# speechbrain/speechbrain

Measured on AMD Instinct MI355X. Metric: audio-sec/s decoded (node), Conformer-L beam=10, higher is better.
Workload: dtype f32

## Files before the change

speechbrain_amd/csrc/gemm.hip:

```cpp
#include "common.h"
#include "internal.h"

#include <map>
#include <mutex>
#include <type_traits>

namespace {

using sbk::f32x16;

#include "gemm_common.h"

__device__ __forceinline__ void tile_epilogue_32x32(const GemmArgs& g, float (&v)[16], int mt, int nt, int r, int half) {
  const int col = nt * 32 + r;
  const bool col_ok = col < g.N;
  const float bv = (g.bias && col_ok) ? g.bias[col] : 0.0f;
  float res[16];
  int len[16];
#pragma unroll
  for (int q = 0; q < 16; ++q) {
    const int row = mt * 32 + (q & 3) + 8 * (q >> 2) + 4 * half;
    const bool live = col_ok && row < g.M;
    res[q] = (live && g.R) ? g.R[(size_t)row * g.ldr + col] : 0.0f;
    len[q] = (live && g.seq_len) ? g.seq_len[row / g.rows_per_seq] : 0x7fffffff;
// ... 936 lines not shown
    } else {
      SBK_LAUNCH((gemm_skinny_flat_kernel<1>), grid, block, 0, st, g, ws, tiles_m, tiles_n);
    }
  } else if (nch >= 4) {
    SBK_LAUNCH((gemm_skinny_kernel<4>), grid, block, 0, st, g, ws, kper, tiles_m, tiles_n);
  } else if (nch >= 2) {
    SBK_LAUNCH((gemm_skinny_kernel<2>), grid, block, 0, st, g, ws, kper, tiles_m, tiles_n);
  } else {
    SBK_LAUNCH((gemm_skinny_kernel<1>), grid, block, 0, st, g, ws, kper, tiles_m, tiles_n);
  }
  int rc = launch_status("gemm_skinny");
  if (rc || SKg == 1) return rc;
  const size_t total = (size_t)M * N;
  SBK_LAUNCH(splitk_reduce_kernel, dim3((unsigned)((total + 1023) / 1024)), dim3(256), 0, st, g, (const float*)ws, SKg);
  return launch_status("splitk_reduce");
}

int gemm_ln_nt(const float* A, int lda, const float* Wf, int ldw, const float* bf, const float* R, int ldr, float* C,
               int ldc, int M, int N, int K, float eps, int act, float alpha, hipStream_t st) {
  if (M == 0 || N == 0) return 0;
  const bool ok = (K == 512 || K == 256 || K == 128) && (M <= 512 || (long)cdiv(M, 128) * cdiv(N, 128) < 256) &&
                  M <= 4096 && (long)M * N < 1900000 && lda % 4 == 0 && ldw % 4 == 0 && aligned16(A) && aligned16(Wf) &&
                  !g_skinny_off;
  if (!ok) return -1;
  GemmArgs g{A, Wf, bf, R, C, lda, ldw, ldr, ldc, M, N, K, act, alpha, nullptr, 1};
  const int tiles_m = cdiv(M, 32), tiles_n = cdiv(N, 32);
  ProfScope prof("gemm_skinny_ln", 2.0 * M * N * K, 4.0 * ((double)M * K + (double)N * K + (double)M * N), st);
  dim3 grid(8 * tiles_m * cdiv(tiles_n, 8)), block(256);
  if (K == 512) {
    SBK_LAUNCH((gemm_skinny_ln_kernel<4>), grid, block, 0, st, g, eps, tiles_m, tiles_n);
  } else if (K == 256) {
    SBK_LAUNCH((gemm_skinny_ln_kernel<2>), grid, block, 0, st, g, eps, tiles_m, tiles_n);
  } else {
    SBK_LAUNCH((gemm_skinny_ln_kernel<1>), grid, block, 0, st, g, eps, tiles_m, tiles_n);
  }
  return launch_status("gemm_skinny_ln");
}

int g_sk_mode = 1;
int g_sk_min_rows = 2048;
namespace {
constexpr int kSkMaxGrid = 512, kSkMaxTiles = 1 << 16;
int sk_cus();
}
int sk_route(int M, int N, int K, int* bt) {
  int unused;
  if (!bt) bt = &unused;
  *bt = 128;
  if (!g_sk_mode || K % 32 != 0 || K < 64) return 0;
  const long T = (long)cdiv(M, 128) * cdiv(N, 128), U = T * (K / 32);
  const int cus = sk_cus();
  int G = 0;
  if (g_sk_mode == 1 && M < g_sk_min_rows) return 0;
  if (g_sk_mode == 1) {
    const bool narrow_short = N <= 512 && K <= 512;
    if (narrow_short ? 2 * T < 3L * cus : U < 16L * cus) return 0;
    G = U >= 32L * cus ? 2 * cus : cus;
  } else {
    if (g_sk_mode == 3 && T < 8) return 0;
    G = 2 * cus;
    if (U / 4 < G) G = (int)(U / 4);
  }
  if (G > kSkMaxGrid) G = kSkMaxGrid;
  return G >= 8 ? (G / 8) * 8 : 8;
}
namespace {
struct SkWorkspace {
  float* slabs;
  int* cnt;
};
std::mutex g_sk_mu;
std::map<std::pair<int, hipStream_t>, SkWorkspace> g_sk_ws;
int g_sk_cus[64] = {};

int cur_device() {
  int dev = 0;
  (void)hipGetDevice(&dev);
  return dev;
}

constexpr size_t kSkSlabBytes = (size_t)2 * 256 * 256 * 256 * sizeof(float);
static_assert(kSkSlabBytes >= (size_t)2 * kSkMaxGrid * 128 * 128 * sizeof(float), "slab area");
constexpr size_t kSkTicketBytes = (size_t)kSkMaxTiles * sizeof(int);

bool sk_workspace(hipStream_t st, SkWorkspace* out) {
  std::lock_guard<std::mutex> lk(g_sk_mu);
  auto it = g_sk_ws.find(std::make_pair(cur_device(), st));
  if (it == g_sk_ws.end()) return false;
  *out = it->second;
  return true;
}

}
int* tile_tickets(hipStream_t st, long tiles) {
  SkWorkspace w;
  if (tiles > kSkMaxTiles || !sk_workspace(st, &w)) return nullptr;
  return w.cnt;
}
bool stream_ws(hipStream_t st, float** slabs, int** cnt) {
  SkWorkspace w;
  if (!sk_workspace(st, &w)) return false;
  *slabs = w.slabs;
  *cnt = w.cnt;
  return true;
}
namespace {

int sk_cus() {
  const int dev = cur_device() & 63;
  if (!g_sk_cus[dev]) {
    int cus = 0;
    (void)hipDeviceGetAttribute(&cus, hipDeviceAttributeMultiprocessorCount, dev);
    g_sk_cus[dev] = cus > 0 ? cus : 256;
  }
  return g_sk_cus[dev];
}

}
int device_cus() { return sk_cus(); }
namespace {
int launch_sk(const GemmArgs& g, int G, int bt, hipStream_t st, bool x3 = false) {
  SkArgs s;
  s.g = g;
  s.tiles_n = cdiv(g.N, bt);
  s.tiles = cdiv(g.M, bt) * s.tiles_n;
  s.KT = g.K / 32;
  if (s.tiles > kSkMaxTiles || (long)s.tiles * s.KT > (1L << 30)) return -1;
  SkWorkspace w;
  if (!sk_workspace(st, &w)) return -1;
  s.slabs = w.slabs;
  s.cnt = w.cnt;
  const size_t lds = x3 ? (size_t)2 * (128 * 32 + 128 * 48) * sizeof(float) : (size_t)(2 * 2 * bt * 32 + 4) * sizeof(float);
  static bool once = false;
  if (!once) {
    (void)SBK_ALLOW_DYN_LDS((gemm_nt_sk_kernel<128, false>), (size_t)(2 * 2 * 128 * 32 + 4) * sizeof(float));
    (void)SBK_ALLOW_DYN_LDS((gemm_nt_sk_kernel<128, true>), (size_t)2 * (128 * 32 + 128 * 48) * sizeof(float));
    once = true;
  }
  const double flops = 2.0 * g.M * g.N * g.K, bytes = 4.0 * ((double)g.M * g.K + (double)g.N * g.K + (double)g.M * g.N);
  if (x3) {
    ProfScope prof("gemm_nt_f32x3", flops, bytes + 2.0 * (double)g.N * g.K, st);
    SBK_LAUNCH((gemm_nt_sk_kernel<128, true>), dim3((unsigned)G), dim3(256), lds, st, s);
  } else {
    ProfScope prof("gemm_nt_persistent", flops, bytes, st);
    SBK_LAUNCH((gemm_nt_sk_kernel<128, false>), dim3((unsigned)G), dim3(256), lds, st, s);
  }
  return launch_status("sbk_gemm_nt_f32 (stream-K)");
}
}

int g_x3_route_rows = 1024, g_x3_route_tiles = 192;
bool x3_routed(int M, int N, int K) {
  return M >= g_x3_route_rows && K % 32 == 0 && K >= 64 && N % 4 == 0 && (long)cdiv(M, 128) * cdiv(N, 128) >= g_x3_route_tiles;
}

int gemm_nt_x3(const float* A, int lda, const uint16_t* W3, const float* bias, const float* R, int ldr, float* C, int ldc,
               int M, int N, int K, int act, float alpha, const int32_t* seq_len, int rows_per_seq, hipStream_t st) {
  if (M == 0 || N == 0) return 0;
  GemmArgs g{A, reinterpret_cast<const float*>(W3), bias, R, C, lda, 0, ldr, ldc, M, N, K, act, alpha, seq_len,
             rows_per_seq > 0 ? rows_per_seq : 1};
  const long T = (long)cdiv(M, 128) * cdiv(N, 128), U = T * (K / 32);
  const int cus = sk_cus();
  int G = T >= 2L * cus ? 2 * cus : cus;
  if (U / 4 < G) G = (int)(U / 4);
  if (G > kSkMaxGrid) G = kSkMaxGrid;
  G = G >= 8 ? (G / 8) * 8 : 8;
  return launch_sk(g, G, 128, st, true);
}

int gemm_nt(const float* A, int lda, const float* W, int ldw, const float* bias, const float* R, int ldr, float* C,
            int ldc, int M, int N, int K, int act, float alpha, const int32_t* seq_len, int rows_per_seq, hipStream_t st) {
  if (M == 0 || N == 0) return 0;
  GemmArgs g{A, W, bias, R, C, lda, ldw, ldr, ldc, M, N, K, act, alpha, seq_len, rows_per_seq > 0 ? rows_per_seq : 1};
  const bool vec = (lda % 4 == 0) && (ldw % 4 == 0) && aligned16(A) && aligned16(W);
  const long tiles128 = (long)cdiv(M, 128) * cdiv(N, 128);
  const long tiles64 = (long)cdiv(M, 64) * cdiv(N, 64);
  if (vec) {
    int bt = 128;
    const int G = sk_route(M, N, K, &bt);
    if (G > 0) {
      const int rc = launch_sk(g, G, bt, st);
      if (rc != -1) return rc;
    }
  }
  if (tiles128 >= 384) return launch_gemm<128, 128, 32, 64, 64>(g, vec, st);
  if (tiles64 >= 256 || M > 256) return launch_gemm<64, 64, 32, 32, 32>(g, vec, st);
  return launch_gemm<32, 64, 32, 32, 32>(g, vec, st);
}
}

extern "C" size_t sbk_stream_workspace_bytes(void) { return sbk::kSkSlabBytes + sbk::kSkTicketBytes; }

extern "C" int sbk_stream_workspace_set(sbk_stream_t stream, void* workspace, size_t workspace_bytes) {
  SBK_REQUIRE(workspace && ((uintptr_t)workspace & 255) == 0, "stream workspace: null or not 256-byte aligned");
  SBK_REQUIRE(workspace_bytes >= sbk_stream_workspace_bytes(), "stream workspace: %zu bytes given, %zu needed", workspace_bytes,
              sbk_stream_workspace_bytes());
  hipStream_t st = sbk::as_stream(stream);
  sbk::SkWorkspace w{reinterpret_cast<float*>(workspace),
                     reinterpret_cast<int*>(reinterpret_cast<char*>(workspace) + sbk::kSkSlabBytes)};
  const hipError_t e = hipMemsetAsync(w.cnt, 0, sbk::kSkTicketBytes, st);
  if (e != hipSuccess) return sbk::fail((int)e, "stream workspace: memset: %s", hipGetErrorString(e));
  std::lock_guard<std::mutex> lk(sbk::g_sk_mu);
  sbk::g_sk_ws[std::make_pair(sbk::cur_device(), st)] = w;
  return 0;
}

extern "C" int sbk_stream_workspace_release(sbk_stream_t stream) {
  std::lock_guard<std::mutex> lk(sbk::g_sk_mu);
  sbk::g_sk_ws.erase(std::make_pair(sbk::cur_device(), sbk::as_stream(stream)));
  return 0;
}

extern "C" int sbk_gemm_nt_f32(const float* A, int lda, const float* W, int ldw, const float* bias,
                               const float* residual, int ldr, float* C, int ldc, int M, int N, int K, int act,
                               float alpha, const int32_t* seq_len, int rows_per_seq, sbk_stream_t stream) {
  if (M == 0 || N == 0) return 0;
  SBK_REQUIRE(A && W && C, "gemm: null operand");
  SBK_REQUIRE(M >= 0 && N >= 0 && K > 0, "gemm: bad shape M=%d N=%d K=%d", M, N, K);
  SBK_REQUIRE(lda > 0 && ldw >= K && ldc >= N, "gemm: leading dimension smaller than the row");
  SBK_REQUIRE(!residual || ldr >= N, "gemm: residual stride");
  SBK_REQUIRE(act >= SBK_ACT_NONE && act <= SBK_ACT_LEAKY_RELU, "gemm: unknown activation %d", act);
  SBK_REQUIRE(!seq_len || rows_per_seq > 0, "gemm: seq_len given without rows_per_seq");
  return sbk::gemm_nt_ws(A, lda, W, ldw, bias, residual, ldr, C, ldc, M, N, K, act, alpha, seq_len, rows_per_seq,
                         nullptr, 0, sbk::as_stream(stream));
}

extern "C" int sbk_gemm_ln_nt_f32(const float* A, int lda, const float* Wf, int ldw, const float* bf,
                                  const float* residual, int ldr, float* C, int ldc, int M, int N, int K, float eps,
                                  int act, float alpha, sbk_stream_t stream) {
  if (M == 0 || N == 0) return 0;
  SBK_REQUIRE(A && Wf && C, "gemm_ln: null operand");
  SBK_REQUIRE(M >= 0 && N >= 0 && K > 0 && lda >= K && ldw >= K && ldc >= N, "gemm_ln: bad shape");
  const int rc = sbk::gemm_ln_nt(A, lda, Wf, ldw, bf, residual, ldr, C, ldc, M, N, K, eps, act, alpha,
                                 sbk::as_stream(stream));
  if (rc == -1) return sbk::fail(SBK_EINVAL, "gemm_ln: shape M=%d N=%d K=%d not eligible for the fused kernel", M, N, K);
  return rc;
}

extern "C" int sbk_gemm_nt_splitk_f32(const float* A, int lda, const float* W, int ldw, const float* bias,
                                      const float* residual, int ldr, float* C, int ldc, int M, int N, int K, int act,
                                      float alpha, float* workspace, size_t workspace_floats, sbk_stream_t stream) {
  if (M == 0 || N == 0) return 0;
  SBK_REQUIRE(A && W && C, "gemm: null operand");
  SBK_REQUIRE(M >= 0 && N >= 0 && K > 0, "gemm: bad shape M=%d N=%d K=%d", M, N, K);
  SBK_REQUIRE(lda >= K && ldw >= K && ldc >= N, "gemm: leading dimension smaller than the row");
  SBK_REQUIRE(!residual || ldr >= N, "gemm: residual stride");
  SBK_REQUIRE(act >= SBK_ACT_NONE && act <= SBK_ACT_LEAKY_RELU, "gemm: unknown activation %d", act);
  return sbk::gemm_nt_ws(A, lda, W, ldw, bias, residual, ldr, C, ldc, M, N, K, act, alpha, nullptr, 0, workspace,
                         workspace ? workspace_floats : 0, sbk::as_stream(stream));
}


extern "C" int sbk_prof_gemm_repeat_f32(const float* A, const float* W, float* C, int M, int N, int K, float* workspace,
                                        size_t workspace_floats, int iters, float* us_per_launch,
                                        sbk_stream_t stream) {
  SBK_REQUIRE(A && W && C && us_per_launch && iters > 0, "gemm_repeat: bad arguments");
  hipStream_t st = sbk::as_stream(stream);
  hipEvent_t e0, e1;
  if (hipEventCreate(&e0) != hipSuccess || hipEventCreate(&e1) != hipSuccess) return sbk::fail(1, "event create");
  int rc = 0;
  for (int i = 0; i < 3 && !rc; ++i)
    rc = sbk::gemm_nt_ws(A, K, W, K, nullptr, nullptr, 0, C, N, M, N, K, SBK_ACT_NONE, 1.0f, nullptr, 0, workspace,
                         workspace_floats, st);
  (void)hipEventRecord(e0, st);
  for (int i = 0; i < iters && !rc; ++i)
    rc = sbk::gemm_nt_ws(A, K, W, K, nullptr, nullptr, 0, C, N, M, N, K, SBK_ACT_NONE, 1.0f, nullptr, 0, workspace,
                         workspace_floats, st);
  (void)hipEventRecord(e1, st);
  (void)hipEventSynchronize(e1);
  float ms = 0.0f;
  (void)hipEventElapsedTime(&ms, e0, e1);
  *us_per_launch = ms * 1000.0f / iters;
  return rc;
}

static int* knob_slot(int key) {
  switch (key) {
    case 2: return &sbk::g_skinny_off;
    case 4: return &sbk::g_cross_rows;
    case 8: return &sbk::g_cross_fc256;
    case 14: return &sbk::g_tiled_splitk;
    case 18: return &sbk::g_sk_mode;
    case 24: return &sbk::g_sk_min_rows;
    case 34: return &sbk::g_x3_route_rows;
    case 35: return &sbk::g_x3_route_tiles;
    case 40: return &sbk::g_score_fused;
    case 41: return &sbk::g_x3r_mode;
    case 42: return &sbk::g_x3r_min_rows;
    case 45: return &sbk::g_x3r_ln;
    case 47: return &sbk::g_persist;
    case 48: return &sbk::g_persist_grid;
    case 49: return &sbk::g_persist_stamps;
    case 51: return &sbk::g_x3r_xc;
    case 53: return &sbk::g_nt_mask;
    case 54: return &sbk::g_x3r_probe;
    case 55: return &sbk::g_self_anc;
    case 58: return &sbk::g_x3r_pair;
    case 59: return &sbk::g_persist_tree;
    case 60: return &sbk::g_attn_exp2;
    case 61: return &sbk::g_lp256;
    case 62: return &sbk::g_lp256_mode;
    case 63: return &sbk::g_x3p_fast_epi;
    case 64: return &sbk::g_x3p_mode;
    default: return nullptr;
  }
}
extern "C" void sbk_prof_set_knob(int key, int value) {
  if (int* p = knob_slot(key)) *p = value;
}
extern "C" int sbk_prof_get_knob(int key) {
  const int* p = knob_slot(key);
  return p ? *p : (-2147483647 - 1);
}


extern "C" int sbk_split_bf16x3(const float* W, int ldw, uint16_t* W3, int N, int K, sbk_stream_t stream) {
  if (N == 0) return 0;
  SBK_REQUIRE(W && W3 && N > 0 && K > 0 && K % 32 == 0 && ldw >= K, "split_bf16x3: bad arguments (K must be a multiple of 32)");
  const long n = (long)N * K, blocks = (n + 255) / 256;
  SBK_LAUNCH(split_bf16x3_kernel, dim3((unsigned)(blocks < 8192 ? blocks : 8192)), dim3(256), 0, sbk::as_stream(stream), W, ldw,
             reinterpret_cast<unsigned short*>(W3), n, K);
  return sbk::launch_status("sbk_split_bf16x3");
}

extern "C" int sbk_gemm_nt_f32x3(const float* A, int lda, const uint16_t* W3, const float* bias, const float* residual,
                                 int ldr, float* C, int ldc, int M, int N, int K, int act, float alpha,
                                 const int32_t* seq_len, int rows_per_seq, sbk_stream_t stream) {
  if (M == 0 || N == 0) return 0;
  SBK_REQUIRE(A && W3 && C, "gemm_f32x3: null operand");
  SBK_REQUIRE(M >= 0 && N >= 0 && K >= 64 && K % 32 == 0, "gemm_f32x3: bad shape M=%d N=%d K=%d (K: a multiple of 32, >= 64)", M, N, K);
  SBK_REQUIRE(lda > 0 && lda % 4 == 0 && ldc >= N && sbk::aligned16(A) && sbk::aligned16(W3),
              "gemm_f32x3: operand rows must be 16-byte aligned (lda=%d)", lda);
  SBK_REQUIRE(N % 4 == 0 && ldc % 4 == 0 && sbk::aligned16(C) && (!bias || sbk::aligned16(bias)),
              "gemm_f32x3: N and ldc must be multiples of 4, C / bias 16-byte aligned (rows are stored as 16-byte vectors)");
  SBK_REQUIRE(!residual || (ldr >= N && ldr % 4 == 0 && sbk::aligned16(residual)), "gemm_f32x3: residual stride / alignment");
  SBK_REQUIRE(act >= SBK_ACT_NONE && act <= SBK_ACT_LEAKY_RELU, "gemm_f32x3: unknown activation %d", act);
  SBK_REQUIRE(!seq_len || rows_per_seq > 0, "gemm_f32x3: seq_len given without rows_per_seq");
  const int rc = sbk::gemm_nt_x3(A, lda, W3, bias, residual, ldr, C, ldc, M, N, K, act, alpha, seq_len, rows_per_seq,
                                 sbk::as_stream(stream));
  if (rc == -1) return sbk::fail(SBK_EINVAL, "gemm_f32x3: no workspace registered for this stream (sbk_stream_workspace_set) or too many tiles");
  return rc;
}
```

speechbrain_amd/csrc/gemm_x3r.hip:

```cpp
#include "common.h"
#include "internal.h"

namespace {

using sbk::f32x16;

struct X3rArgs {
  const float* A;
  const uint4* PW;
  const float* bias;
  const float* R;
  float* C;
  int ns;
  int lda, ldr, ldc, M, N, K, act, tiles_m, tiles_n;
  float alpha;
  float ln_eps;
  int xc;
};

template <int NS, int LNQ = 0, bool PAIR = false>
__global__ void __launch_bounds__(256, 2) gemm_x3r_kernel(X3rArgs g) {
  constexpr int DEPTH = 4, PD = 3;
  __shared__ float4 red[4][4][4][64];
  __shared__ float2 stat[LNQ > 0 ? 64 : 1];
  const int lane = threadIdx.x & 63, wave = threadIdx.x >> 6;
  int nt, mt;
  {
    const int id = blockIdx.x, x = id & 7, q = id >> 3;
    const int c = g.xc, r = 8 / c, rm = (g.tiles_m + r - 1) / r;
    mt = x / c + r * (q % rm);
    nt = x % c + c * (q / rm);
    if (mt >= g.tiles_m || nt >= g.tiles_n) return;
  }
  const int r = lane & 31, half = lane >> 5;
  const int ns = NS > 0 ? NS : g.ns, k_begin = wave * ns * 16, KB = g.K >> 4;
  const float* arow[2];
#pragma unroll
  for (int i = 0; i < 2; ++i) arow[i] = g.A + (size_t)min(mt * 64 + i * 32 + r, g.M - 1) * g.lda + k_begin + 8 * half;
  const uint4* wp = g.PW + ((size_t)(nt * KB + (k_begin >> 4)) * 6 + half) * 64 + r;
  float4 av[DEPTH][2][2];
  uint4 wv[DEPTH][2][3];
  auto load = [&](int buf, int st) SBK_INLINE_LAMBDA {
#pragma unroll
    for (int j = 0; j < 2; ++j)
#pragma unroll
      for (int p = 0; p < 3; ++p) wv[buf][j][p] = wp[(size_t)st * 384 + p * 128 + j * 32];
#pragma unroll
    for (int i = 0; i < 2; ++i) {
      av[buf][i][0] = *reinterpret_cast<const float4*>(arow[i] + st * 16);
      av[buf][i][1] = *reinterpret_cast<const float4*>(arow[i] + st * 16 + 4);
    }
  };
  f32x16 acc[2][2];
#pragma unroll
  for (int i = 0; i < 2; ++i)
#pragma unroll
    for (int j = 0; j < 2; ++j)
#pragma unroll
      for (int q = 0; q < 16; ++q) acc[i][j][q] = 0.0f;
  float mean[2] = {0.0f, 0.0f};
  auto compute = [&](int buf) SBK_INLINE_LAMBDA {
    sbk::bf16x8 ap[2][3], bp[2][3];
#pragma unroll
    for (int j = 0; j < 2; ++j)
#pragma unroll
      for (int p = 0; p < 3; ++p) {
        sbk::pin(wv[buf][j][p].x), sbk::pin(wv[buf][j][p].y), sbk::pin(wv[buf][j][p].z), sbk::pin(wv[buf][j][p].w);
        const uint4 u = wv[buf][j][p];
        bp[j][p] = sbk::bf16x8_from_words(u.x, u.y, u.z, u.w);
      }
#pragma unroll
    for (int i = 0; i < 2; ++i) {
#pragma unroll
      for (int e = 0; e < 2; ++e) {
        sbk::pin(av[buf][i][e].x), sbk::pin(av[buf][i][e].y), sbk::pin(av[buf][i][e].z), sbk::pin(av[buf][i][e].w);
      }
      const float4 x0 = av[buf][i][0], x1 = av[buf][i][1];
      float x[8] = {x0.x, x0.y, x0.z, x0.w, x1.x, x1.y, x1.z, x1.w};
      if constexpr (LNQ > 0) {
#pragma unroll
        for (int e = 0; e < 8; ++e) x[e] -= mean[i];
      }
      unsigned h[4], m[4], l[4];
#pragma unroll
      for (int p = 0; p < 4; ++p) {
        h[p] = sbk::bf16_pair(x[2 * p], x[2 * p + 1]);
        const float r0 = x[2 * p] - __uint_as_float(h[p] << 16), r1 = x[2 * p + 1] - __uint_as_float(h[p] & 0xffff0000u);
        m[p] = sbk::bf16_pair(r0, r1);
        l[p] = sbk::bf16_pair(r0 - __uint_as_float(m[p] << 16), r1 - __uint_as_float(m[p] & 0xffff0000u));
      }
      ap[i][0] = sbk::bf16x8_from_words(h[0], h[1], h[2], h[3]);
      ap[i][1] = sbk::bf16x8_from_words(m[0], m[1], m[2], m[3]);
      ap[i][2] = sbk::bf16x8_from_words(l[0], l[1], l[2], l[3]);
    }
    constexpr int PA_[6] = {2, 0, 1, 1, 0, 0}, PB_[6] = {0, 2, 1, 0, 1, 0};
#pragma unroll
    for (int t = 0; t < 6; ++t)
#pragma unroll
      for (int i = 0; i < 2; ++i)
#pragma unroll
        for (int j = 0; j < 2; ++j) acc[i][j] = sbk::mfma_32x32x16_bf16(bp[j][PB_[t]], ap[i][PA_[t]], acc[i][j]);
  };
#pragma unroll
  for (int st = 0; st < (PAIR ? DEPTH : PD); ++st) load(st, st);
  if constexpr (LNQ > 0) {
    const float inv_k = 1.0f / (float)g.K;
    const int grp = lane >> 4, t = lane & 15;
#pragma unroll
    for (int ps = 0; ps < 4; ++ps) {
      const int rl = wave * 16 + ps * 4 + grp;
      const float4* xr = reinterpret_cast<const float4*>(g.A + (size_t)min(mt * 64 + rl, g.M - 1) * g.lda);
      float4 xs[4 * LNQ];
#pragma unroll
      for (int j = 0; j < 4 * LNQ; ++j) xs[j] = xr[t + 16 * j];
      float sm = 0.0f;
#pragma unroll
      for (int j = 0; j < 4 * LNQ; ++j) sm += (xs[j].x + xs[j].y) + (xs[j].z + xs[j].w);
      const float mu = sbk::group_sum<16>(sm) * inv_k;
      float qs = 0.0f;
#pragma unroll
      for (int j = 0; j < 4 * LNQ; ++j) {
        const float a = xs[j].x - mu, b = xs[j].y - mu, c = xs[j].z - mu, d = xs[j].w - mu;
        qs += (a * a + b * b) + (c * c + d * d);
      }
      const float rs = rsqrtf(sbk::group_sum<16>(qs) * inv_k + g.ln_eps);
      if (t == 0) stat[rl] = make_float2(mu, rs);
    }
    __syncthreads();
#pragma unroll
    for (int i = 0; i < 2; ++i) mean[i] = stat[i * 32 + r].x;
  }
  if constexpr (PAIR && NS > 0) {
#pragma unroll
    for (int st = 0; st < NS; st += 2) {
      compute(st % DEPTH);
      compute((st + 1) % DEPTH);
      sbk::sched_fence();
      if (st + DEPTH < NS) {
        load(st % DEPTH, st + DEPTH);
        load((st + 1) % DEPTH, st + DEPTH + 1);
      }
      sbk::sched_fence();
    }
  } else if constexpr (PAIR) {
#pragma unroll 1
    for (int s0 = 0; s0 < ns; s0 += DEPTH) {
#pragma unroll
      for (int j = 0; j < DEPTH; j += 2) {
        compute(j);
        compute(j + 1);
        sbk::sched_fence();
        if (s0 + j + DEPTH < ns) {
          load(j, s0 + j + DEPTH);
          load(j + 1, s0 + j + DEPTH + 1);
        }
        sbk::sched_fence();
      }
    }
  } else if constexpr (NS > 0) {
#pragma unroll
    for (int st = 0; st < NS; ++st) {
      if (st + PD < NS) load((st + PD) % DEPTH, st + PD);
      sbk::sched_fence();
      compute(st % DEPTH);
    }
  } else {
#pragma unroll 1
    for (int s0 = 0; s0 < ns; s0 += DEPTH) {
#pragma unroll
      for (int j = 0; j < DEPTH; ++j) {
        if (s0 + j + PD < ns) load((j + PD) % DEPTH, s0 + j + PD);
        sbk::sched_fence();
        compute(j);
      }
    }
  }
  const int row = (mt * 2 + (wave >> 1)) * 32 + r, col0 = (nt * 2 + (wave & 1)) * 32 + 4 * half;
  const bool row_ok = row < g.M;
  const float* rrow = g.R ? g.R + (size_t)(row_ok ? row : 0) * g.ldr : nullptr;
  float4 bv[4], rv[4];
  bool ok[4];
  auto side_loads = [&]() SBK_INLINE_LAMBDA {
#pragma unroll
    for (int q4 = 0; q4 < 4; ++q4) {
      const int col = col0 + 8 * q4;
      ok[q4] = row_ok && col < g.N;
      bv[q4] = (g.bias && ok[q4]) ? *reinterpret_cast<const float4*>(g.bias + col) : make_float4(0.0f, 0.0f, 0.0f, 0.0f);
      rv[q4] = (rrow && ok[q4]) ? *reinterpret_cast<const float4*>(rrow + col) : make_float4(0.0f, 0.0f, 0.0f, 0.0f);
    }
  };
  side_loads();
#pragma unroll
  for (int i = 0; i < 2; ++i)
#pragma unroll
    for (int j = 0; j < 2; ++j)
#pragma unroll
      for (int q4 = 0; q4 < 4; ++q4)
        red[wave][2 * i + j][q4][lane] = make_float4(acc[i][j][4 * q4], acc[i][j][4 * q4 + 1], acc[i][j][4 * q4 + 2], acc[i][j][4 * q4 + 3]);
  __syncthreads();
  float4 v[4];
#pragma unroll
  for (int q4 = 0; q4 < 4; ++q4) {
    const float4 a0 = red[0][wave][q4][lane], a1 = red[1][wave][q4][lane], a2 = red[2][wave][q4][lane], a3 = red[3][wave][q4][lane];
    v[q4] = make_float4(((a0.x + a1.x) + a2.x) + a3.x, ((a0.y + a1.y) + a2.y) + a3.y, ((a0.z + a1.z) + a2.z) + a3.z,
                        ((a0.w + a1.w) + a2.w) + a3.w);
  }
  if constexpr (LNQ > 0) {
    const float rs = stat[(wave >> 1) * 32 + r].y;
#pragma unroll
    for (int q4 = 0; q4 < 4; ++q4) v[q4].x *= rs, v[q4].y *= rs, v[q4].z *= rs, v[q4].w *= rs;
  }
  float o[16];
#pragma unroll
  for (int q4 = 0; q4 < 4; ++q4) {
    o[4 * q4] = v[q4].x + bv[q4].x, o[4 * q4 + 1] = v[q4].y + bv[q4].y, o[4 * q4 + 2] = v[q4].z + bv[q4].z, o[4 * q4 + 3] = v[q4].w + bv[q4].w;
  }
  switch (g.act) {
    case SBK_ACT_SWISH:
#pragma unroll
      for (int q = 0; q < 16; ++q) o[q] = o[q] / (1.0f + expf(-o[q]));
      break;
    case SBK_ACT_GELU:
#pragma unroll
      for (int q = 0; q < 16; ++q) o[q] = 0.5f * o[q] * (1.0f + erff(o[q] * 0.70710678118654752440f));
      break;
    case SBK_ACT_RELU:
#pragma unroll
      for (int q = 0; q < 16; ++q) o[q] = o[q] > 0.0f ? o[q] : 0.0f;
      break;
    case SBK_ACT_LEAKY_RELU:
#pragma unroll
      for (int q = 0; q < 16; ++q) o[q] = o[q] > 0.0f ? o[q] : 0.01f * o[q];
      break;
    default: break;
  }
#pragma unroll
  for (int q4 = 0; q4 < 4; ++q4) {
    const int col = col0 + 8 * q4;
    const float o0 = o[4 * q4] * g.alpha + rv[q4].x, o1 = o[4 * q4 + 1] * g.alpha + rv[q4].y;
    const float o2 = o[4 * q4 + 2] * g.alpha + rv[q4].z, o3 = o[4 * q4 + 3] * g.alpha + rv[q4].w;
    if (!ok[q4]) continue;
    *reinterpret_cast<float4*>(g.C + (size_t)row * g.ldc + col) = make_float4(o0, o1, o2, o3);
  }
}

__global__ void __launch_bounds__(256) x3r_touch_kernel(const uint4* __restrict__ p, size_t n16, unsigned* __restrict__ sink) {
  const size_t per = (n16 + 31) / 32, b0 = (size_t)(blockIdx.x >> 3) * per, b1 = b0 + per < n16 ? b0 + per : n16;
  unsigned acc = 0;
  for (size_t i = b0 + threadIdx.x; i < b1; i += 256) {
    const uint4 v = p[i];
    acc ^= v.x ^ v.y ^ v.z ^ v.w;
  }
  if (acc == 0x9e3779b9u && n16 == 1) *sink = acc;
}

}

namespace sbk {

int g_x3r_mode = 2;
int g_x3r_min_rows = 192;
bool x3r_routed(int M, int N, int K) { return g_x3r_mode != 0 && M >= g_x3r_min_rows && K % 256 == 0 && N % 4 == 0; }
int g_x3r_ln = 1;
int g_x3r_pair = 1;
int g_x3r_probe = 0;
int g_x3r_xc = 0;

static int launch_x3r(const float* A, int lda, const uint16_t* PW, const float* bias, const float* R, int ldr, float* C, int ldc,
                      int M, int N, int K, int act, float alpha, float ln_eps, hipStream_t st) {
  if (M == 0 || N == 0) return 0;
  const bool ln = ln_eps >= 0.0f;
  if (K % 256 != 0 || N % 4 != 0 || !aligned16(PW) || !A || !C || lda % 4 != 0 || !aligned16(A)) return -1;
  if (ldc % 4 != 0 || !aligned16(C) || (R && (ldr % 4 != 0 || !aligned16(R))) || (bias && !aligned16(bias))) return -1;
  if (ln && !(K == 256 || K == 512 || K == 1024 || K == 1280)) return -1;
  const int tm = cdiv(M, 64), tn = cdiv(N, 64);
  int xc = g_x3r_xc;
  if (!(xc == 1 || xc == 2 || xc == 4 || xc == 8)) {
    const double ab = 4.0 * M * (double)K, wb = 6.0 * N * (double)K;
    xc = 8;
    for (int c = 4; c >= 1; c >>= 1)
      if (c * ab + (8 / c) * wb < xc * ab + (8 / xc) * wb) xc = c;
  }
  X3rArgs a{A, reinterpret_cast<const uint4*>(PW), bias, R, C, K / 64, lda, ldr, ldc, M, N, K, act, tm, tn, alpha, ln_eps, xc};
  if (g_x3r_probe >= 2) {
    ProfScope pt("x3r_touch", 0.0, 8.0 * 6.0 * (double)N * K, st);
    SBK_LAUNCH(x3r_touch_kernel, dim3(256), dim3(256), 0, st, reinterpret_cast<const uint4*>(PW), (size_t)N * K * 6 / 16, (unsigned*)nullptr);
    if (g_x3r_probe == 3 && lda == K)
      SBK_LAUNCH(x3r_touch_kernel, dim3(256), dim3(256), 0, st, reinterpret_cast<const uint4*>(A), (size_t)M * K * 4 / 16, (unsigned*)nullptr);
  }
  const int reps = g_x3r_probe == 1 ? 2 : 1;
  int rc_last = 0;
  for (int rep = 0; rep < reps; ++rep) {
  ProfScope prof(rep ? (ln ? "gemm_ln_x3r_rep" : "gemm_x3r_rep") : (ln ? "gemm_ln_x3r" : "gemm_x3r"), 2.0 * M * N * K,
                 4.0 * M * (double)K + 6.0 * (double)N * K + (4.0 + (R ? 4.0 : 0.0)) * M * (double)N, st);
  dim3 grid(8 * cdiv(tm, 8 / xc) * cdiv(tn, xc)), block(256);
  const int pair = g_x3r_pair;
  if (ln) {
    if (K == 512) {
      if (pair & 2) SBK_LAUNCH((gemm_x3r_kernel<8, 2, true>), grid, block, 0, st, a);
      else SBK_LAUNCH((gemm_x3r_kernel<8, 2>), grid, block, 0, st, a);
    } else if (K == 256) {
      SBK_LAUNCH((gemm_x3r_kernel<4, 1>), grid, block, 0, st, a);
    } else if (K == 1024) {
      SBK_LAUNCH((gemm_x3r_kernel<0, 4>), grid, block, 0, st, a);
    } else {
      SBK_LAUNCH((gemm_x3r_kernel<0, 5>), grid, block, 0, st, a);
    }
    rc_last = launch_status("gemm_ln_x3r");
  } else {
    if (K == 512 && N >= 1024 && g_x3r_mode != 3) {
      if (pair & 1) SBK_LAUNCH((gemm_x3r_kernel<8, 0, true>), grid, block, 0, st, a);
      else SBK_LAUNCH((gemm_x3r_kernel<8>), grid, block, 0, st, a);
    } else {
      if (pair & 1) SBK_LAUNCH((gemm_x3r_kernel<0, 0, true>), grid, block, 0, st, a);
      else SBK_LAUNCH((gemm_x3r_kernel<0>), grid, block, 0, st, a);
    }
    rc_last = launch_status("gemm_x3r");
  }
  if (rc_last) return rc_last;
  }
  return rc_last;
}
int gemm_nt_x3r(const float* A, int lda, const uint16_t* PW, const float* bias, const float* R, int ldr, float* C, int ldc, int M,
                int N, int K, int act, float alpha, hipStream_t st) {
  return launch_x3r(A, lda, PW, bias, R, ldr, C, ldc, M, N, K, act, alpha, -1.0f, st);
}
int gemm_ln_nt_x3r(const float* A, int lda, const uint16_t* PWf, const float* bf, const float* R, int ldr, float* C, int ldc, int M,
                   int N, int K, float eps, int act, float alpha, hipStream_t st) {
  if (!(eps >= 0.0f)) return -1;
  return launch_x3r(A, lda, PWf, bf, R, ldr, C, ldc, M, N, K, act, alpha, eps, st);
}
bool x3r_ln_routed(int K) { return g_x3r_ln != 0 && (K == 256 || K == 512 || K == 1024 || K == 1280); }

}

extern "C" int sbk_gemm_nt_x3r(const float* A, int lda, const uint16_t* PW, const float* bias, const float* residual, int ldr,
                               float* C, int ldc, int M, int N, int K, int act, float alpha, sbk_stream_t stream) {
  if (M == 0 || N == 0) return 0;
  SBK_REQUIRE(A && PW && C, "gemm_x3r: null operand");
  SBK_REQUIRE(M >= 0 && N >= 0 && N % 4 == 0 && K >= 256 && K % 256 == 0,
              "gemm_x3r: bad shape M=%d N=%d K=%d (N: a multiple of 4, K: a multiple of 256)", M, N, K);
  SBK_REQUIRE(lda >= K && lda % 4 == 0 && sbk::aligned16(A), "gemm_x3r: rows of A must be 16-byte aligned (lda=%d)", lda);
  SBK_REQUIRE(sbk::aligned16(PW), "gemm_x3r: the panel image must be 16-byte aligned");
  SBK_REQUIRE(ldc >= N && ldc % 4 == 0 && sbk::aligned16(C), "gemm_x3r: C rows are stored as 16-byte vectors (ldc=%d)", ldc);
  SBK_REQUIRE(!residual || (ldr >= N && ldr % 4 == 0 && sbk::aligned16(residual)), "gemm_x3r: residual stride / alignment");
  SBK_REQUIRE(!bias || sbk::aligned16(bias), "gemm_x3r: bias alignment");
  SBK_REQUIRE(act >= SBK_ACT_NONE && act <= SBK_ACT_LEAKY_RELU, "gemm_x3r: unknown activation %d", act);
  const int rc = sbk::gemm_nt_x3r(A, lda, PW, bias, residual, ldr, C, ldc, M, N, K, act, alpha, sbk::as_stream(stream));
  if (rc == -1) return sbk::fail(SBK_EINVAL, "gemm_x3r: shape not eligible");
  return rc;
}

extern "C" int sbk_gemm_ln_nt_x3r(const float* A, int lda, const uint16_t* PWf, const float* bf, const float* residual, int ldr,
                                  float* C, int ldc, int M, int N, int K, float eps, int act, float alpha, sbk_stream_t stream) {
  if (M == 0 || N == 0) return 0;
  SBK_REQUIRE(A && PWf && C, "gemm_ln_x3r: null operand");
  SBK_REQUIRE(M >= 0 && N >= 0 && N % 4 == 0 && (K == 256 || K == 512 || K == 1024 || K == 1280),
              "gemm_ln_x3r: bad shape M=%d N=%d K=%d (N: a multiple of 4, K: 256, 512, 1024 or 1280)", M, N, K);
  SBK_REQUIRE(eps >= 0.0f, "gemm_ln_x3r: eps must be >= 0");
  SBK_REQUIRE(lda >= K && lda % 4 == 0 && sbk::aligned16(A), "gemm_ln_x3r: rows of A must be 16-byte aligned (lda=%d)", lda);
  SBK_REQUIRE(sbk::aligned16(PWf), "gemm_ln_x3r: the panel image must be 16-byte aligned");
  SBK_REQUIRE(ldc >= N && ldc % 4 == 0 && sbk::aligned16(C), "gemm_ln_x3r: C rows are stored as 16-byte vectors (ldc=%d)", ldc);
  SBK_REQUIRE(!residual || (ldr >= N && ldr % 4 == 0 && sbk::aligned16(residual)), "gemm_ln_x3r: residual stride / alignment");
  SBK_REQUIRE(!bf || sbk::aligned16(bf), "gemm_ln_x3r: bias alignment");
  SBK_REQUIRE(act >= SBK_ACT_NONE && act <= SBK_ACT_LEAKY_RELU, "gemm_ln_x3r: unknown activation %d", act);
  const int rc = sbk::gemm_ln_nt_x3r(A, lda, PWf, bf, residual, ldr, C, ldc, M, N, K, eps, act, alpha, sbk::as_stream(stream));
  if (rc == -1) return sbk::fail(SBK_EINVAL, "gemm_ln_x3r: shape not eligible");
  return rc;
}
```

speechbrain_amd/csrc/internal.h:

```cpp
#pragma once
#include "common.h"

namespace sbk {
int gemm_nt(const float* A, int lda, const float* W, int ldw, const float* bias, const float* R, int ldr, float* C,
            int ldc, int M, int N, int K, int act, float alpha, const int32_t* seq_len, int rows_per_seq,
            hipStream_t st);
int gemm_nt_x3(const float* A, int lda, const uint16_t* W3, const float* bias, const float* R, int ldr, float* C, int ldc,
               int M, int N, int K, int act, float alpha, const int32_t* seq_len, int rows_per_seq, hipStream_t st);
bool x3_routed(int M, int N, int K);
int gemm_nt_x3p(const uint16_t* PA, const uint16_t* PW, const float* bias, const float* R, int ldr, float* C, int ldc,
                uint16_t* PC, int M, int N, int K, int act, float alpha, const int32_t* seq_len, int rows_per_seq, hipStream_t st);
int gemm_nt_x3r(const float* A, int lda, const uint16_t* PW, const float* bias, const float* R, int ldr, float* C, int ldc, int M,
                int N, int K, int act, float alpha, hipStream_t st);
bool x3r_routed(int M, int N, int K);
int gemm_ln_nt_x3r(const float* A, int lda, const uint16_t* PWf, const float* bf, const float* R, int ldr, float* C, int ldc, int M,
                   int N, int K, float eps, int act, float alpha, hipStream_t st);
bool x3r_ln_routed(int K);
extern int g_x3r_mode, g_x3r_min_rows, g_x3r_ln, g_x3r_probe, g_x3r_pair;
bool persist_eligible(const sbk_decoder_weights* W, int n, int B, int beam, int Lmax);
int persist_barriers(int n_layers);
int decoder_step_persist(const sbk_decoder_weights* W, const int32_t* tokens, const int32_t* kv_slot, const int32_t* enc_len,
                         float* x, float* qkv, float* ctx, float* q, float* ff, float* h, float* logits, float* const* kcache,
                         float* const* vcache, float* const* ckv, int* bar, int bar_seq, int* grid_io, int step, int n, int B, int T,
                         int beam, int Lmax, bool want_logits, hipStream_t st);
extern int g_persist, g_persist_grid, g_persist_stamps, g_persist_tree;
extern thread_local const int32_t* g_step_ptr;
extern thread_local int g_step_min_steps;
extern int g_cross_rows;
extern int g_nt_mask;
extern int g_self_anc;
extern int g_attn_exp2;
extern int g_cross_fc256;
struct Lp256Args {
  const unsigned char* A;
  const unsigned char* W;
  const float* sa;
  const float* sw;
  const float* bias;
  const float* R;
  float* C;
  unsigned short* Cb;
  unsigned char* C8;
  float c8_scale;
  long lda, ldw;
  int ldr, ldc, ldcb, ldc8, M, N, act;
  float alpha;
  int KT, tiles_m, tiles_n, tiles, whole;
};
bool lp256_routed(const Lp256Args& a);
int gemm_nt_lp256(const Lp256Args& a, bool fp8, hipStream_t st);
extern int g_lp256, g_lp256_mode, g_x3p_mode, g_x3p_fast_epi;
extern int g_x3r_xc;
extern int g_score_fused;
constexpr float kCtcNeg = -1e20f;
__device__ __forceinline__ float ls_logit(float x, float b1, float b2, float inv_temp) {
  return mul_rn(add_rn(add_rn(x, b1), b2), inv_temp);
}
__device__ __forceinline__ float ls_out(float v, float lse, float w) { return mul_rn(w, sub_rn(v, lse)); }
__device__ __forceinline__ float score_ctc(float v, float psi, float psi_prev, float weight) {
  return add_rn(v, mul_rn(sub_rn(psi, psi_prev), weight));
}
__device__ __forceinline__ float score_cand(float seq, float comb, float norm) {
  const float x = add_rn(seq, comb);
  return norm > 0.0f ? x / norm : x;
}
int gemm_nt_ws(const float* A, int lda, const float* W, int ldw, const float* bias, const float* R, int ldr, float* C,
               int ldc, int M, int N, int K, int act, float alpha, const int32_t* seq_len, int rows_per_seq, float* ws,
               size_t ws_floats, hipStream_t st);
int gemm_ln_nt(const float* A, int lda, const float* Wf, int ldw, const float* bf, const float* R, int ldr, float* C,
               int ldc, int M, int N, int K, float eps, int act, float alpha, hipStream_t st);
int layernorm(const float* x, const float* gamma, const float* beta, float* y, int rows, int d, float eps, int act,
              hipStream_t st);
int relpos_attention(const float* qkv, const float* pos, const float* bias_u, const float* bias_v,
                     const int32_t* key_len, float* out, float* attn, int B, int T, int H, int Dh, float scale,
                     hipStream_t st, int chunk = 0, int left = -1);
int glu_dwconv(const float* h, const float* w, const float* bias, float* y, int B, int T, int d, int ksize,
               hipStream_t st, int chunk = 0);
}
```

Before: 13270.

## Add 32-row tile variant to x3r GEMM for small grids, plus ablation knobs

Templates the bf16x3 split-precision GEMM kernel on tile height, adding a 32-row variant. It is chosen by default when the 32-row tile count is at most 256, which raises the number of workgroups for the small-M decoder GEMMs. The epilogue is generalised so each wave reduces and stores a variable number of quads. It also adds compile-time ablation variants (skip MFMA, loads, exchange, epilogue, stats) behind a knob; these are off by default and exist only for profiling. Smaller tiles mean more weight re-reads per output and less MFMA reuse per block.

After: 13310, median of 6. Within noise of the previous version (+0.2%).

```diff
diff --git a/speechbrain_amd/csrc/gemm.hip b/speechbrain_amd/csrc/gemm.hip
--- a/speechbrain_amd/csrc/gemm.hip
+++ b/speechbrain_amd/csrc/gemm.hip
@@ -1262,6 +1262,8 @@
     case 62: return &sbk::g_lp256_mode;
     case 63: return &sbk::g_x3p_fast_epi;
     case 64: return &sbk::g_x3p_mode;
+    case 67: return &sbk::g_x3r_tile;
+    case 68: return &sbk::g_x3r_abl;
     default: return nullptr;
   }
 }
diff --git a/speechbrain_amd/csrc/gemm_x3r.hip b/speechbrain_amd/csrc/gemm_x3r.hip
--- a/speechbrain_amd/csrc/gemm_x3r.hip
+++ b/speechbrain_amd/csrc/gemm_x3r.hip
@@ -18,11 +18,15 @@
   int xc;
 };
 
-template <int NS, int LNQ = 0, bool PAIR = false>
+template <int NS, int LNQ = 0, bool PAIR = false, int MT = 64, int ABL = 0>
 __global__ void __launch_bounds__(256, 2) gemm_x3r_kernel(X3rArgs g) {
   constexpr int DEPTH = 4, PD = 3;
-  __shared__ float4 red[4][4][4][64];
-  __shared__ float2 stat[LNQ > 0 ? 64 : 1];
+  static_assert(MT == 64 || MT == 32, "gemm_x3r: 64- or 32-row tiles");
+  constexpr int RI = MT / 32;
+  constexpr bool kNoMfma = ABL & 1, kNoA = ABL & 2, kNoW = ABL & 4, kNoXchg = ABL & 8, kNoEpi = ABL & 16, kNoStat = ABL & 32,
+                 kEmpty = ABL & 64;
+  __shared__ float4 red[4][2 * RI][4][64];
+  __shared__ float2 stat[LNQ > 0 ? MT : 1];
   const int lane = threadIdx.x & 63, wave = threadIdx.x >> 6;
   int nt, mt;
   {
@@ -32,35 +36,42 @@
     nt = x % c + c * (q / rm);
     if (mt >= g.tiles_m || nt >= g.tiles_n) return;
   }
+  if constexpr (kEmpty) return;
   const int r = lane & 31, half = lane >> 5;
   const int ns = NS > 0 ? NS : g.ns, k_begin = wave * ns * 16, KB = g.K >> 4;
-  const float* arow[2];
-#pragma unroll
-  for (int i = 0; i < 2; ++i) arow[i] = g.A + (size_t)min(mt * 64 + i * 32 + r, g.M - 1) * g.lda + k_begin + 8 * half;
+  const float* arow[RI];
+#pragma unroll
+  for (int i = 0; i < RI; ++i) arow[i] = g.A + (size_t)min(mt * MT + i * 32 + r, g.M - 1) * g.lda + k_begin + 8 * half;
   const uint4* wp = g.PW + ((size_t)(nt * KB + (k_begin >> 4)) * 6 + half) * 64 + r;
-  float4 av[DEPTH][2][2];
+  float4 av[DEPTH][RI][2];
   uint4 wv[DEPTH][2][3];
   auto load = [&](int buf, int st) SBK_INLINE_LAMBDA {
 #pragma unroll
     for (int j = 0; j < 2; ++j)
 #pragma unroll
-      for (int p = 0; p < 3; ++p) wv[buf][j][p] = wp[(size_t)st * 384 + p * 128 + j * 32];
-#pragma unroll
-    for (int i = 0; i < 2; ++i) {
-      av[buf][i][0] = *reinterpret_cast<const float4*>(arow[i] + st * 16);
-      av[buf][i][1] = *reinterpret_cast<const float4*>(arow[i] + st * 16 + 4);
+      for (int p = 0; p < 3; ++p) wv[buf][j][p] = kNoW ? make_uint4(0u, 0u, 0u, 0u) : wp[(size_t)st * 384 + p * 128 + j * 32];
+#pragma unroll
+    for (int i = 0; i < RI; ++i) {
+      if constexpr (kNoA) {
+        av[buf][i][0] = av[buf][i][1] = make_float4(0.0f, 0.0f, 0.0f, 0.0f);
+      } else {
+        av[buf][i][0] = *reinterpret_cast<const float4*>(arow[i] + st * 16);
+        av[buf][i][1] = *reinterpret_cast<const float4*>(arow[i] + st * 16 + 4);
+      }
     }
   };
-  f32x16 acc[2][2];
-#pragma unroll
-  for (int i = 0; i < 2; ++i)
+  f32x16 acc[RI][2];
+#pragma unroll
+  for (int i = 0; i < RI; ++i)
 #pragma unroll
     for (int j = 0; j < 2; ++j)
 #pragma unroll
       for (int q = 0; q < 16; ++q) acc[i][j][q] = 0.0f;
-  float mean[2] = {0.0f, 0.0f};
+  float mean[RI];
+#pragma unroll
+  for (int i = 0; i < RI; ++i) mean[i] = 0.0f;
   auto compute = [&](int buf) SBK_INLINE_LAMBDA {
-    sbk::bf16x8 ap[2][3], bp[2][3];
+    sbk::bf16x8 ap[RI][3], bp[2][3];
 #pragma unroll
     for (int j = 0; j < 2; ++j)
 #pragma unroll
@@ -70,7 +81,7 @@
         bp[j][p] = sbk::bf16x8_from_words(u.x, u.y, u.z, u.w);
       }
 #pragma unroll
-    for (int i = 0; i < 2; ++i) {
+    for (int i = 0; i < RI; ++i) {
 #pragma unroll
       for (int e = 0; e < 2; ++e) {
         sbk::pin(av[buf][i][e].x), sbk::pin(av[buf][i][e].y), sbk::pin(av[buf][i][e].z), sbk::pin(av[buf][i][e].w);
@@ -88,28 +99,35 @@
         const float r0 = x[2 * p] - __uint_as_float(h[p] << 16), r1 = x[2 * p + 1] - __uint_as_float(h[p] & 0xffff0000u);
         m[p] = sbk::bf16_pair(r0, r1);
         l[p] = sbk::bf16_pair(r0 - __uint_as_float(m[p] << 16), r1 - __uint_as_float(m[p] & 0xffff0000u));
+        if constexpr (kNoMfma) sbk::pin(h[p]), sbk::pin(m[p]), sbk::pin(l[p]);
       }
       ap[i][0] = sbk::bf16x8_from_words(h[0], h[1], h[2], h[3]);
       ap[i][1] = sbk::bf16x8_from_words(m[0], m[1], m[2], m[3]);
       ap[i][2] = sbk::bf16x8_from_words(l[0], l[1], l[2], l[3]);
     }
     constexpr int PA_[6] = {2, 0, 1, 1, 0, 0}, PB_[6] = {0, 2, 1, 0, 1, 0};
+    if constexpr (kNoMfma) return;
 #pragma unroll
     for (int t = 0; t < 6; ++t)
 #pragma unroll
-      for (int i = 0; i < 2; ++i)
+      for (int i = 0; i < RI; ++i)
 #pragma unroll
         for (int j = 0; j < 2; ++j) acc[i][j] = sbk::mfma_32x32x16_bf16(bp[j][PB_[t]], ap[i][PA_[t]], acc[i][j]);
   };
 #pragma unroll
   for (int st = 0; st < (PAIR ? DEPTH : PD); ++st) load(st, st);
-  if constexpr (LNQ > 0) {
+  if constexpr (LNQ > 0 && kNoStat) {
+    if (threadIdx.x < MT) stat[threadIdx.x] = make_float2(0.0f, 1.0f);
+    __syncthreads();
+#pragma unroll
+    for (int i = 0; i < RI; ++i) mean[i] = stat[i * 32 + r].x;
+  } else if constexpr (LNQ > 0) {
     const float inv_k = 1.0f / (float)g.K;
     const int grp = lane >> 4, t = lane & 15;
 #pragma unroll
-    for (int ps = 0; ps < 4; ++ps) {
-      const int rl = wave * 16 + ps * 4 + grp;
-      const float4* xr = reinterpret_cast<const float4*>(g.A + (size_t)min(mt * 64 + rl, g.M - 1) * g.lda);
+    for (int ps = 0; ps < MT / 16; ++ps) {
+      const int rl = wave * (MT / 4) + ps * 4 + grp;
+      const float4* xr = reinterpret_cast<const float4*>(g.A + (size_t)min(mt * MT + rl, g.M - 1) * g.lda);
       float4 xs[4 * LNQ];
 #pragma unroll
       for (int j = 0; j < 4 * LNQ; ++j) xs[j] = xr[t + 16 * j];
@@ -128,7 +146,7 @@
     }
     __syncthreads();
 #pragma unroll
-    for (int i = 0; i < 2; ++i) mean[i] = stat[i * 32 + r].x;
+    for (int i = 0; i < RI; ++i) mean[i] = stat[i * 32 + r].x;
   }
   if constexpr (PAIR && NS > 0) {
 #pragma unroll
@@ -175,71 +193,99 @@
       }
     }
   }
-  const int row = (mt * 2 + (wave >> 1)) * 32 + r, col0 = (nt * 2 + (wave & 1)) * 32 + 4 * half;
+  if constexpr (ABL != 0) {
+#pragma unroll
+    for (int i = 0; i < RI; ++i)
+#pragma unroll
+      for (int j = 0; j < 2; ++j) sbk::pin(acc[i][j]);
+  }
+  constexpr int NQ = 2 * RI;
+  const int s0 = (wave * NQ) >> 2, qb = (wave * NQ) & 3, si = s0 >> 1, sj = s0 & 1;
+  const int row = (mt * RI + si) * 32 + r, col0 = (nt * 2 + sj) * 32 + 4 * half + 8 * qb;
   const bool row_ok = row < g.M;
   const float* rrow = g.R ? g.R + (size_t)(row_ok ? row : 0) * g.ldr : nullptr;
-  float4 bv[4], rv[4];
-  bool ok[4];
+  float4 bv[NQ], rv[NQ];
+  bool ok[NQ];
   auto side_loads = [&]() SBK_INLINE_LAMBDA {
 #pragma unroll
-    for (int q4 = 0; q4 < 4; ++q4) {
-      const int col = col0 + 8 * q4;
-      ok[q4] = row_ok && col < g.N;
-      bv[q4] = (g.bias && ok[q4]) ? *reinterpret_cast<const float4*>(g.bias + col) : make_float4(0.0f, 0.0f, 0.0f, 0.0f);
-      rv[q4] = (rrow && ok[q4]) ? *reinterpret_cast<const float4*>(rrow + col) : make_float4(0.0f, 0.0f, 0.0f, 0.0f);
+    for (int q = 0; q < NQ; ++q) {
+      const int col = col0 + 8 * q;
+      ok[q] = row_ok && col < g.N;
+      bv[q] = (g.bias && ok[q]) ? *reinterpret_cast<const float4*>(g.bias + col) : make_float4(0.0f, 0.0f, 0.0f, 0.0f);
+      rv[q] = (rrow && ok[q]) ? *reinterpret_cast<const float4*>(rrow + col) : make_float4(0.0f, 0.0f, 0.0f, 0.0f);
     }
   };
-  side_loads();
-#pragma unroll
-  for (int i = 0; i < 2; ++i)
-#pragma unroll
-    for (int j = 0; j < 2; ++j)
-#pragma unroll
-      for (int q4 = 0; q4 < 4; ++q4)
-        red[wave][2 * i + j][q4][lane] = make_float4(acc[i][j][4 * q4], acc[i][j][4 * q4 + 1], acc[i][j][4 * q4 + 2], acc[i][j][4 * q4 + 3]);
-  __syncthreads();
-  float4 v[4];
-#pragma unroll
-  for (int q4 = 0; q4 < 4; ++q4) {
-    const float4 a0 = red[0][wave][q4][lane], a1 = red[1][wave][q4][lane], a2 = red[2][wave][q4][lane], a3 = red[3][wave][q4][lane];
-    v[q4] = make_float4(((a0.x + a1.x) + a2.x) + a3.x, ((a0.y + a1.y) + a2.y) + a3.y, ((a0.z + a1.z) + a2.z) + a3.z,
-                        ((a0.w + a1.w) + a2.w) + a3.w);
+  if constexpr (!kNoEpi) side_loads();
+  float4 v[NQ];
+  if constexpr (kNoXchg) {
+#pragma unroll
+    for (int q = 0; q < NQ; ++q) v[q] = make_float4(0.0f, 0.0f, 0.0f, 0.0f);
+#pragma unroll
+    for (int i = 0; i < RI; ++i)
+#pragma unroll
+      for (int j = 0; j < 2; ++j)
+#pragma unroll
+        for (int q4 = 0; q4 < 4; ++q4)
+#pragma unroll
+          for (int q = 0; q < NQ; ++q)
+            if (i == si && j == sj && q4 == qb + q)
+              v[q] = make_float4(acc[i][j][4 * q4], acc[i][j][4 * q4 + 1], acc[i][j][4 * q4 + 2], acc[i][j][4 * q4 + 3]);
+  } else {
+#pragma unroll
+    for (int i = 0; i < RI; ++i)
+#pragma unroll
+      for (int j = 0; j < 2; ++j)
+#pragma unroll
+        for (int q4 = 0; q4 < 4; ++q4)
+          red[wave][2 * i + j][q4][lane] = make_float4(acc[i][j][4 * q4], acc[i][j][4 * q4 + 1], acc[i][j][4 * q4 + 2], acc[i][j][4 * q4 + 3]);
+    __syncthreads();
+#pragma unroll
+    for (int q = 0; q < NQ; ++q) {
+      const float4 a0 = red[0][s0][qb + q][lane], a1 = red[1][s0][qb + q][lane], a2 = red[2][s0][qb + q][lane], a3 = red[3][s0][qb + q][lane];
+      v[q] = make_float4(((a0.x + a1.x) + a2.x) + a3.x, ((a0.y + a1.y) + a2.y) + a3.y, ((a0.z + a1.z) + a2.z) + a3.z,
+                         ((a0.w + a1.w) + a2.w) + a3.w);
+    }
+  }
+  if constexpr (kNoEpi) {
+#pragma unroll
+    for (int q = 0; q < NQ; ++q) sbk::pin(v[q].x), sbk::pin(v[q].y), sbk::pin(v[q].z), sbk::pin(v[q].w);
+    return;
   }
   if constexpr (LNQ > 0) {
-    const float rs = stat[(wave >> 1) * 32 + r].y;
-#pragma unroll
-    for (int q4 = 0; q4 < 4; ++q4) v[q4].x *= rs, v[q4].y *= rs, v[q4].z *= rs, v[q4].w *= rs;
-  }
-  float o[16];
-#pragma unroll
-  for (int q4 = 0; q4 < 4; ++q4) {
-    o[4 * q4] = v[q4].x + bv[q4].x, o[4 * q4 + 1] = v[q4].y + bv[q4].y, o[4 * q4 + 2] = v[q4].z + bv[q4].z, o[4 * q4 + 3] = v[q4].w + bv[q4].w;
+    const float rs = stat[si * 32 + r].y;
+#pragma unroll
+    for (int q = 0; q < NQ; ++q) v[q].x *= rs, v[q].y *= rs, v[q].z *= rs, v[q].w *= rs;
+  }
+  float o[4 * NQ];
+#pragma unroll
+  for (int q = 0; q < NQ; ++q) {
+    o[4 * q] = v[q].x + bv[q].x, o[4 * q + 1] = v[q].y + bv[q].y, o[4 * q + 2] = v[q].z + bv[q].z, o[4 * q + 3] = v[q].w + bv[q].w;
   }
   switch (g.act) {
     case SBK_ACT_SWISH:
 #pragma unroll
-      for (int q = 0; q < 16; ++q) o[q] = o[q] / (1.0f + expf(-o[q]));
+      for (int q = 0; q < 4 * NQ; ++q) o[q] = o[q] / (1.0f + expf(-o[q]));
       break;
     case SBK_ACT_GELU:
 #pragma unroll
-      for (int q = 0; q < 16; ++q) o[q] = 0.5f * o[q] * (1.0f + erff(o[q] * 0.70710678118654752440f));
+      for (int q = 0; q < 4 * NQ; ++q) o[q] = 0.5f * o[q] * (1.0f + erff(o[q] * 0.70710678118654752440f));
       break;
     case SBK_ACT_RELU:
 #pragma unroll
-      for (int q = 0; q < 16; ++q) o[q] = o[q] > 0.0f ? o[q] : 0.0f;
+      for (int q = 0; q < 4 * NQ; ++q) o[q] = o[q] > 0.0f ? o[q] : 0.0f;
       break;
     case SBK_ACT_LEAKY_RELU:
 #pragma unroll
-      for (int q = 0; q < 16; ++q) o[q] = o[q] > 0.0f ? o[q] : 0.01f * o[q];
+      for (int q = 0; q < 4 * NQ; ++q) o[q] = o[q] > 0.0f ? o[q] : 0.01f * o[q];
       break;
     default: break;
   }
 #pragma unroll
-  for (int q4 = 0; q4 < 4; ++q4) {
-    const int col = col0 + 8 * q4;
-    const float o0 = o[4 * q4] * g.alpha + rv[q4].x, o1 = o[4 * q4 + 1] * g.alpha + rv[q4].y;
-    const float o2 = o[4 * q4 + 2] * g.alpha + rv[q4].z, o3 = o[4 * q4 + 3] * g.alpha + rv[q4].w;
-    if (!ok[q4]) continue;
+  for (int q = 0; q < NQ; ++q) {
+    const int col = col0 + 8 * q;
+    const float o0 = o[4 * q] * g.alpha + rv[q].x, o1 = o[4 * q + 1] * g.alpha + rv[q].y;
+    const float o2 = o[4 * q + 2] * g.alpha + rv[q].z, o3 = o[4 * q + 3] * g.alpha + rv[q].w;
+    if (!ok[q]) continue;
     *reinterpret_cast<float4*>(g.C + (size_t)row * g.ldc + col) = make_float4(o0, o1, o2, o3);
   }
 }
@@ -265,6 +311,31 @@
 int g_x3r_pair = 1;
 int g_x3r_probe = 0;
 int g_x3r_xc = 0;
+int g_x3r_tile = 1;
+int g_x3r_abl = 0;
+
+template <int NS, int LNQ, bool PAIR, int MT>
+static void launch_x3r_kernel(dim3 grid, hipStream_t st, const X3rArgs& a) {
+  constexpr bool kAbl = (NS == 0 || NS == 8) && ((LNQ == 0 && PAIR) || (LNQ == 2 && !PAIR));
+  if constexpr (kAbl) {
+    switch (g_x3r_abl) {
+      case 1: SBK_LAUNCH((gemm_x3r_kernel<NS, LNQ, PAIR, MT, 1>), grid, dim3(256), 0, st, a); return;
+      case 2: SBK_LAUNCH((gemm_x3r_kernel<NS, LNQ, PAIR, MT, 2>), grid, dim3(256), 0, st, a); return;
+      case 4: SBK_LAUNCH((gemm_x3r_kernel<NS, LNQ, PAIR, MT, 4>), grid, dim3(256), 0, st, a); return;
+      case 8: SBK_LAUNCH((gemm_x3r_kernel<NS, LNQ, PAIR, MT, 8>), grid, dim3(256), 0, st, a); return;
+      case 16: SBK_LAUNCH((gemm_x3r_kernel<NS, LNQ, PAIR, MT, 16>), grid, dim3(256), 0, st, a); return;
+      case 32:
+        if constexpr (LNQ > 0) {
+          SBK_LAUNCH((gemm_x3r_kernel<NS, LNQ, PAIR, MT, 32>), grid, dim3(256), 0, st, a);
+          return;
+        }
+        break;
+      case 64: SBK_LAUNCH((gemm_x3r_kernel<NS, LNQ, PAIR, MT, 64>), grid, dim3(256), 0, st, a); return;
+      default: break;
+    }
+  }
+  SBK_LAUNCH((gemm_x3r_kernel<NS, LNQ, PAIR, MT>), grid, dim3(256), 0, st, a);
+}
 
 static int launch_x3r(const float* A, int lda, const uint16_t* PW, const float* bias, const float* R, int ldr, float* C, int ldc,
                       int M, int N, int K, int act, float alpha, float ln_eps, hipStream_t st) {
@@ -273,7 +344,8 @@
   if (K % 256 != 0 || N % 4 != 0 || !aligned16(PW) || !A || !C || lda % 4 != 0 || !aligned16(A)) return -1;
   if (ldc % 4 != 0 || !aligned16(C) || (R && (ldr % 4 != 0 || !aligned16(R))) || (bias && !aligned16(bias))) return -1;
   if (ln && !(K == 256 || K == 512 || K == 1024 || K == 1280)) return -1;
-  const int tm = cdiv(M, 64), tn = cdiv(N, 64);
+  const bool t32 = g_x3r_tile != 0 && (long)cdiv(M, 32) * cdiv(N, 64) <= 256;
+  const int tm = cdiv(M, t32 ? 32 : 64), tn = cdiv(N, 64);
   int xc = g_x3r_xc;
   if (!(xc == 1 || xc == 2 || xc == 4 || xc == 8)) {
     const double ab = 4.0 * M * (double)K, wb = 6.0 * N * (double)K;
@@ -297,23 +369,41 @@
   const int pair = g_x3r_pair;
   if (ln) {
     if (K == 512) {
-      if (pair & 2) SBK_LAUNCH((gemm_x3r_kernel<8, 2, true>), grid, block, 0, st, a);
-      else SBK_LAUNCH((gemm_x3r_kernel<8, 2>), grid, block, 0, st, a);
+      if (pair & 2) {
+        if (t32) launch_x3r_kernel<8, 2, true, 32>(grid, st, a);
+        else launch_x3r_kernel<8, 2, true, 64>(grid, st, a);
+      } else {
+        if (t32) launch_x3r_kernel<8, 2, false, 32>(grid, st, a);
+        else launch_x3r_kernel<8, 2, false, 64>(grid, st, a);
+      }
     } else if (K == 256) {
-      SBK_LAUNCH((gemm_x3r_kernel<4, 1>), grid, block, 0, st, a);
+      if (t32) launch_x3r_kernel<4, 1, false, 32>(grid, st, a);
+      else launch_x3r_kernel<4, 1, false, 64>(grid, st, a);
     } else if (K == 1024) {
-      SBK_LAUNCH((gemm_x3r_kernel<0, 4>), grid, block, 0, st, a);
+      if (t32) launch_x3r_kernel<0, 4, false, 32>(grid, st, a);
+      else launch_x3r_kernel<0, 4, false, 64>(grid, st, a);
     } else {
-      SBK_LAUNCH((gemm_x3r_kernel<0, 5>), grid, block, 0, st, a);
+      if (t32) launch_x3r_kernel<0, 5, false, 32>(grid, st, a);
+      else launch_x3r_kernel<0, 5, false, 64>(grid, st, a);
     }
     rc_last = launch_status("gemm_ln_x3r");
   } else {
     if (K == 512 && N >= 1024 && g_x3r_mode != 3) {
-      if (pair & 1) SBK_LAUNCH((gemm_x3r_kernel<8, 0, true>), grid, block, 0, st, a);
-      else SBK_LAUNCH((gemm_x3r_kernel<8>), grid, block, 0, st, a);
+      if (pair & 1) {
+        if (t32) launch_x3r_kernel<8, 0, true, 32>(grid, st, a);
+        else launch_x3r_kernel<8, 0, true, 64>(grid, st, a);
+      } else {
+        if (t32) launch_x3r_kernel<8, 0, false, 32>(grid, st, a);
+        else launch_x3r_kernel<8, 0, false, 64>(grid, st, a);
+      }
     } else {
-      if (pair & 1) SBK_LAUNCH((gemm_x3r_kernel<0, 0, true>), grid, block, 0, st, a);
-      else SBK_LAUNCH((gemm_x3r_kernel<0>), grid, block, 0, st, a);
+      if (pair & 1) {
+        if (t32) launch_x3r_kernel<0, 0, true, 32>(grid, st, a);
+        else launch_x3r_kernel<0, 0, true, 64>(grid, st, a);
+      } else {
+        if (t32) launch_x3r_kernel<0, 0, false, 32>(grid, st, a);
+        else launch_x3r_kernel<0, 0, false, 64>(grid, st, a);
+      }
     }
     rc_last = launch_status("gemm_x3r");
   }
diff --git a/speechbrain_amd/csrc/internal.h b/speechbrain_amd/csrc/internal.h
--- a/speechbrain_amd/csrc/internal.h
+++ b/speechbrain_amd/csrc/internal.h
@@ -50,7 +50,7 @@
 bool lp256_routed(const Lp256Args& a);
 int gemm_nt_lp256(const Lp256Args& a, bool fp8, hipStream_t st);
 extern int g_lp256, g_lp256_mode, g_x3p_mode, g_x3p_fast_epi;
-extern int g_x3r_xc;
+extern int g_x3r_xc, g_x3r_tile, g_x3r_abl;
 extern int g_score_fused;
 constexpr float kCtcNeg = -1e20f;
 __device__ __forceinline__ float ls_logit(float x, float b1, float b2, float inv_temp) {
```
